# nyrahealth/CrisperWhisper

Hardware: AMD Instinct MI355X
Metric: aligned words/s (RTF alongside), CrisperWhisper large-v3 geometry, 30 s chunks, full mel->encoder->decoder->DTW->words path (higher is better)
Workload: dtype bf16

## Files before the change

crisperwhisper_amd/csrc/common.h:

```cpp
#pragma once
#include <hip/hip_runtime.h>
#include <stdint.h>
#include <stdio.h>
#include <math.h>

typedef unsigned short bf16_t;

typedef __attribute__((ext_vector_type(8))) short bf16x8_t;
typedef __attribute__((ext_vector_type(4))) float f32x4_t;

#define CW_WAVE 64

#ifdef CW_NO_NT
#define CW_STREAM_LD(p) (*(p))
#else
#define CW_STREAM_LD(p) __builtin_nontemporal_load(p)
#endif

static inline float cw_host_bf16_to_f32(unsigned short v) { union { uint32_t u; float f; } x; x.u = ((uint32_t)v) << 16; return x.f; }
static inline unsigned short cw_host_f32_to_bf16(float f) {
    union { uint32_t u; float f; } x; x.f = f;
    const uint32_t rounded = (x.u + 0x7fffu + ((x.u >> 16) & 1u)) >> 16;
    const uint32_t nan = (x.u >> 16) | 0x40u;
    return (unsigned short)(((x.u & 0x7fffffffu) > 0x7f800000u) ? nan : rounded);
// ... 268 lines not shown
        Pack4<T>::st((T*)p.out + (size_t)m * p.ldo + n, a0, a1, a2, a3);
    } else if (MODE == EPI_GELU) {
        Pack4<T>::st((T*)p.out + (size_t)m * p.ldo + n, Pack4<T>::gelu(a0), Pack4<T>::gelu(a1), Pack4<T>::gelu(a2), Pack4<T>::gelu(a3));
    } else if (MODE == EPI_RESID_F32) {
        const size_t o = (size_t)m * p.ldo + n;
        const float4 r = *(const float4*)(p.resid + o);
        *(float4*)(p.outf + o) = make_float4(r.x + a0, r.y + a1, r.z + a2, r.w + a3);
    } else if (MODE == EPI_GELU_POS_F32) {
        const float4 ps = *(const float4*)(p.pos + (size_t)(m % p.T) * p.ldo + n);
        *(float4*)(p.outf + (size_t)m * p.ldo + n) =
            make_float4(Pack4<T>::gelu(a0) + ps.x, Pack4<T>::gelu(a1) + ps.y, Pack4<T>::gelu(a2) + ps.z, Pack4<T>::gelu(a3) + ps.w);
    } else if (MODE == EPI_HEADS) {
        const int which = n / p.d_model, r = n - which * p.d_model;
        const int h = r >> 6, dd = r & 63;
        const int b = m / p.T, s = m - b * p.T;
        T* base = (T*)(which == 0 ? p.out : (which == 1 ? p.out1 : p.out2));
        Pack4<T>::st(base + (((size_t)b * p.H + h) * p.S_pad + s) * 64 + dd, a0, a1, a2, a3);
    } else if (MODE == EPI_STORE_F32) {
        *(float4*)(p.outf + (size_t)m * p.ldo + n) = make_float4(a0, a1, a2, a3);
    }
}

template <typename T, int MODE>
__device__ inline void epi_tile_interior(const EpiParams& p, const int (&rows)[4], const int (&cols)[4],
                                         const f32x4_t (&acc)[4][4]) {
    size_t roff[4]; int rpos[4];
    float4 bias[4]; size_t coff[4]; T* cbase[4];
#pragma unroll
    for (int i = 0; i < 4; ++i) {
        const int m = rows[i];
        rpos[i] = 0;
        if (MODE == EPI_HEADS) {
            const int b = m / p.T, s_ = m - b * p.T;
            roff[i] = ((size_t)b * p.H * p.S_pad + s_) * 64;
        } else {
            roff[i] = (size_t)m * p.ldo;
            if (MODE == EPI_GELU_POS_F32) rpos[i] = m % p.T;
        }
    }
#pragma unroll
    for (int j = 0; j < 4; ++j) {
        const int n = cols[j];
        bias[j] = p.bias ? *(const float4*)(p.bias + n) : make_float4(0.f, 0.f, 0.f, 0.f);
        cbase[j] = (T*)p.out;
        if (MODE == EPI_HEADS) {
            const int which = n / p.d_model, r = n - which * p.d_model;
            cbase[j] = (T*)(which == 0 ? p.out : (which == 1 ? p.out1 : p.out2));
            coff[j] = (size_t)(r >> 6) * p.S_pad * 64 + (r & 63);
        } else {
            coff[j] = (size_t)n;
        }
    }
#pragma unroll
    for (int i = 0; i < 4; ++i)
#pragma unroll
        for (int j = 0; j < 4; ++j) {
            const float a0 = acc[i][j][0] + bias[j].x, a1 = acc[i][j][1] + bias[j].y;
            const float a2 = acc[i][j][2] + bias[j].z, a3 = acc[i][j][3] + bias[j].w;
            const size_t o = roff[i] + coff[j];
            if (MODE == EPI_STORE || MODE == EPI_HEADS) {
                Pack4<T>::st(cbase[j] + o, a0, a1, a2, a3);
            } else if (MODE == EPI_GELU) {
                Pack4<T>::st(cbase[j] + o, Pack4<T>::gelu(a0), Pack4<T>::gelu(a1), Pack4<T>::gelu(a2), Pack4<T>::gelu(a3));
            } else if (MODE == EPI_RESID_F32) {
                const float4 r = *(const float4*)(p.resid + o);
                *(float4*)(p.outf + o) = make_float4(r.x + a0, r.y + a1, r.z + a2, r.w + a3);
            } else if (MODE == EPI_GELU_POS_F32) {
                const float4 ps = *(const float4*)(p.pos + (size_t)rpos[i] * p.ldo + cols[j]);
                *(float4*)(p.outf + o) = make_float4(Pack4<T>::gelu(a0) + ps.x, Pack4<T>::gelu(a1) + ps.y,
                                                     Pack4<T>::gelu(a2) + ps.z, Pack4<T>::gelu(a3) + ps.w);
            } else if (MODE == EPI_STORE_F32) {
                *(float4*)(p.outf + o) = make_float4(a0, a1, a2, a3);
            }
        }
}

#define CW_OK 0
#define CW_ERR_INVALID (-22)
#define CW_ERR_NOMEM (-12)
#define CW_ERR_HIP (-5)
#define CW_ERR_STATE (-1)
#define CW_TOP_LOGPROBS_MAX 8
```

crisperwhisper_amd/csrc/engine.hip:

```cpp
#include <chrono>
#include <hip/hip_runtime.h>
#include <stdarg.h>
#include <stdlib.h>
#include <string.h>
#include <set>
#include <string>
#include <vector>
#include <functional>
#include <algorithm>

#include "../../include/crisperwhisper.h"
#include "kernels.h"

static thread_local char g_err[512] = "";

#define KD(c, fn, ...) ((c)->f16 ? cw_f16::fn(__VA_ARGS__) : cw_bf16::fn(__VA_ARGS__))

#define CW_MAX_DEC_STAGES 24
enum DecStageKind { DST_OTHER = 0, DST_QKV_SELF, DST_QKV, DST_SELF_ATTN, DST_O_PROJ, DST_STACK, DST_STACK_CROSS, DST_CROSS_Q, DST_CROSS_ATTN,
                    DST_CROSS_O, DST_FC1, DST_FC2, DST_MLP_PAIR, DST_MLP_CHAIN, DST_N };
static const char* const kDecStageName[DST_N] = {
    "other (A/B path)", "LayerNorm + q/k/v projection + self-attention (qkv_self_kernel)", "LayerNorm + q/k/v projection + cache append",
    "self-attention", "self-attention out-projection", "fused out-projection + cross-query stage (gemv_stack_kernel)",
    "fused stage + cross-attention (dec_layer_a_kernel)", "LayerNorm + cross-attention query projection", "cross-attention",
// ... 50 lines not shown
    bool mid16 = true;
    bool dtw_block = false;
    bool stack_center = true;
    int skinny_mode = 0;
    float* d_planes = nullptr;
    size_t planes_cap = 0;
    float* d_sk_stats = nullptr;
    float* d_rstats = nullptr;
    bool fuse6_enabled = true;
    bool fuse_mlp = false;
    bool mlp_pair_fence = false;
    bool mlp_pair = false;
    unsigned int* d_bar = nullptr; int* d_err = nullptr;
    int handoff_fallbacks = 0;
    int handoff_resumes = 0;
    long long forwards_since_reset = 0;
    int fail_pos = -1;
    bool declayer = false;
    bool qkv_self = true;
    unsigned long long *d_gq = nullptr, *d_gps = nullptr, *d_gq2 = nullptr, *d_gkv = nullptr, *d_gflag = nullptr;
    bool mlp_chain = false;
    unsigned int* d_epoch = nullptr;
    int n_cu = 0;
    int stack_nt3 = 0, stack_nt5 = 0;
    bool ln_folded = false;
    bool fold_enabled = true;
    std::set<std::string> loaded;
    bool weights_ok = false;
    bool wpacked = false;
    bool wpack_enabled = true;
    void* embed_pk = nullptr;

    void *conv1_w = nullptr, *conv2_w = nullptr, *embed = nullptr;
    float *conv1_b = nullptr, *conv2_b = nullptr, *enc_pos = nullptr, *dec_pos = nullptr;
    float *enc_ln_g = nullptr, *enc_ln_b = nullptr, *dec_ln_g = nullptr, *dec_ln_b = nullptr;
    std::vector<LayerW> enc, dec;

    MelTables mel{};
    float *d_pcm = nullptr, *d_logspec = nullptr, *d_feats_hf = nullptr;
    unsigned int* d_gmax = nullptr;
    void* d_feats_tm = nullptr;
    std::vector<int> n_frames_items;

    void *c1 = nullptr, *h = nullptr, *qb = nullptr, *kb = nullptr, *vb = nullptr, *ao = nullptr, *mid = nullptr,
         *enc_out = nullptr;
    float* x = nullptr;
// ... 561 lines not shown
        "model.encoder.embed_positions.weight", "model.encoder.layer_norm.weight", "model.encoder.layer_norm.bias",
        "model.decoder.embed_tokens.weight", "model.decoder.embed_positions.weight", "model.decoder.layer_norm.weight",
        "model.decoder.layer_norm.bias"};
    auto attn = [&](const std::string& p) {
        for (const char* t : {".q_proj.weight", ".q_proj.bias", ".k_proj.weight", ".v_proj.weight", ".v_proj.bias",
                              ".out_proj.weight", ".out_proj.bias"}) want.push_back(p + t);
    };
    auto pair = [&](const std::string& p) { want.push_back(p + ".weight"); want.push_back(p + ".bias"); };
    for (int stack = 0; stack < 2; ++stack) {
        const int nl = stack ? c->d.dec_layers : c->d.enc_layers;
        for (int l = 0; l < nl; ++l) {
            const std::string p = std::string(stack ? "model.decoder.layers." : "model.encoder.layers.") + std::to_string(l);
            attn(p + ".self_attn"); pair(p + ".self_attn_layer_norm");
            if (stack) { attn(p + ".encoder_attn"); pair(p + ".encoder_attn_layer_norm"); }
            pair(p + ".fc1"); pair(p + ".fc2"); pair(p + ".final_layer_norm");
        }
    }
    std::string missing; int n_missing = 0;
    for (const auto& w : want)
        if (!c->loaded.count(w)) { if (n_missing < 4) missing += (n_missing ? ", " : "") + w; ++n_missing; }
    if (n_missing) return fail(c, CW_ERR_STATE, "%d of %zu weight tensors were never loaded (e.g. %s): incomplete checkpoint", n_missing, want.size(), missing.c_str());
    CWCHK(c, apply_folds(c));
    CWCHK(c, pack_decoder_weights(c));
    c->weights_ok = true;
    return CW_OK;
}

static int stage_fold(cw_ctx* c, int layer, int which, const float* data, int N, int K, void* w_dst, size_t w_off, float* b_dst,
                      size_t b_off, float scale) {
    cw_ctx::Fold f{nullptr, N, K, w_dst, w_off, b_dst, b_off, scale, layer, which};
    HIPCHK(c, hipMalloc((void**)&f.stage, (size_t)N * K * 4));
    HIPCHK(c, hipMemcpy(f.stage, data, (size_t)N * K * 4, hipMemcpyHostToDevice));
    c->folds.push_back(f);
    return CW_OK;
}

static int apply_folds(cw_ctx* c) {
    for (auto& f : c->folds) {
        LayerW& L = c->dec[f.layer];
        const float* g = f.which == 0 ? L.ln1_g : (f.which == 1 ? L.lnc_g : L.ln2_g);
        const float* b = f.which == 0 ? L.ln1_b : (f.which == 1 ? L.lnc_b : L.ln2_b);
        CWCHK(c, KD(c, cw_launch_fold_layernorm, f.stage, f.N, f.K, g, b, f.scale, (bf16_t*)f.w_dst + f.w_off, f.b_dst + f.b_off, c->st));
    }
    const int D = c->d.d_model, F = c->d.ffn_dim;
    bool all = !c->folds.empty() && c->fuse6_enabled && F % D == 0 && D <= 1280 && D % 64 == 0 && F % 64 == 0 && c->d.n_heads <= 20;
    if (all) {
// ... 287 lines not shown
        }
        if (c->enc8_mask & 2) CWCHK(c, KD(c, cw_launch_layernorm_fp8, c->x, L.ln2_g, L.ln2_b, c->h8, c->sa8, M, D, c->st));
        else CWCHK(c, KD(c, cw_launch_layernorm, bf, c->x, L.ln2_g, L.ln2_b, c->h, M, D, c->st));
        {
            AParams ap{c->h, D, 0, 0, 0, 0, nullptr, nullptr};
            EpiParams ep = epi0(); ep.out = c->mid; ep.bias = L.b1; ep.ldo = F;
            if (c->enc8_mask & 2) CWCHK(c, KD(c, cw_launch_gemm_fp8, EPI_GELU, c->h8, D, L.w18, M, F, D, c->sa8, L.s1, ep, c->st));
            else CWCHK(c, KD(c, cw_launch_gemm, bf, EPI_GELU, ap, L.w1, M, F, D, ep, c->st));
        }
        {
            AParams ap{c->mid, F, 0, 0, 0, 0, nullptr, nullptr};
            EpiParams ep = epi0(); ep.outf = c->x; ep.resid = c->x; ep.bias = L.b2; ep.ldo = D;
            if (c->enc8_mask & 4) {
                CWCHK(c, KD(c, cw_launch_quant_rows_fp8, c->mid, M, F, c->mid8, c->smid8, c->st));
                CWCHK(c, KD(c, cw_launch_gemm_fp8, EPI_RESID_F32, c->mid8, F, L.w28, M, D, F, c->smid8, L.s2, ep, c->st));
            } else CWCHK(c, KD(c, cw_launch_gemm, bf, EPI_RESID_F32, ap, L.w2, M, D, F, ep, c->st));
        }
    }
    CWCHK(c, KD(c, cw_launch_layernorm, bf, c->x, c->enc_ln_g, c->enc_ln_b, c->enc_out, M, D, c->st));
    if (c->enc8_mask & 8) CWCHK(c, KD(c, cw_launch_layernorm_fp8, c->x, c->enc_ln_g, c->enc_ln_b, c->h8, c->sa8, M, D, c->st));
    KCHK(c);
    tm.stop();
    StageTimer tk(c, CW_STAGE_CROSS_KV);
    for (int l = 0; l < c->d.dec_layers; ++l) {
        LayerW& L = c->dec[l];
        AParams ap{c->enc_out, D, 0, 0, 0, 0, nullptr, nullptr};
        EpiParams ep = epi0(); ep.out = L.ck; ep.out1 = L.cv; ep.bias = L.bkv_c;
        ep.T = S; ep.S_pad = S; ep.H = H; ep.d_model = D;
        if (c->enc8_mask & 8) CWCHK(c, KD(c, cw_launch_gemm_fp8, EPI_HEADS, c->h8, D, L.wkv_c8, M, 2 * D, D, c->sa8, L.skv_c, ep, c->st));
        else CWCHK(c, KD(c, cw_launch_gemm, bf, EPI_HEADS, ap, L.wkv_c, M, 2 * D, D, ep, c->st));
        if (c->kv8) CWCHK(c, KD(c, cw_launch_kv_quant_fp8, L.ck, L.cv, L.ck8, L.cv8, L.kvs, nb, H, S, c->st));
    }
    KCHK(c);
    tk.stop();
    c->nb_encoded = nb;
    return CW_OK;
}

int32_t cw_get_encoder_output(cw_ctx* c, float* out, int32_t nb) {
    if (nb < 1 || nb > c->nb_encoded) return fail(c, CW_ERR_STATE, "only %d windows encoded", c->nb_encoded);
    HIPCHK(c, hipStreamSynchronize(c->st));
    return download_T(c, c->enc_out, 0, out, (size_t)nb * CW_N_CTX * c->d.d_model);
}

static int gemv_ln(cw_ctx* c, int epi, const float* x, int Mb, int K, const void* W, int N, const float* g,
                   const float* b, const EpiParams& ep) {
    if (c->bf16 || !g) return KD(c, cw_launch_gemv, c->bf16, epi, x, Mb, K, W, N, g, b, ep, c->st, nullptr, (Mb <= 16 || c->wpacked) ? c->d_xfrag : nullptr, c->bf16 && c->wpacked);
// ... 1976 lines not shown
        for (auto& ge : c->step_graph) if (ge) { hipGraphExecDestroy(ge); ge = nullptr; }
        return CW_OK;
    }
    return fail(c, CW_ERR_INVALID, "unknown option %s", name);
}

int32_t cw_has_experiments(void) {
#ifdef CW_EXPERIMENTS
    return 1;
#else
    return 0;
#endif
}

static int g_test_cross_fp8 = 0;
static int g_test_attn_poison_qpad = 0;
int32_t cw_test_set_option(const char* name, int32_t value) {
    if (!strcmp(name, "cross_test_fp8")) { g_test_cross_fp8 = value; return CW_OK; }
    if (!strcmp(name, "attn_poison_qpad")) { g_test_attn_poison_qpad = value; return CW_OK; }
    if (!strcmp(name, "gemm256_min_tiles")) { cw_bf16::cw_gemm_set_256_min_tiles(value); cw_f16::cw_gemm_set_256_min_tiles(value); return CW_OK; }
    if (!strcmp(name, "beam_topk_1block")) { cw_bf16::cw_beam_topk_set_1block(value); cw_f16::cw_beam_topk_set_1block(value); return CW_OK; }
    if (!strcmp(name, "gemm_pp")) { cw_bf16::cw_gemm_set_pp(value); cw_f16::cw_gemm_set_pp(value); return CW_OK; }
    if (!strcmp(name, "gemm_8ph")) { cw_bf16::cw_gemm_set_8ph(value); cw_f16::cw_gemm_set_8ph(value); return CW_OK; }
    if (!strcmp(name, "gemm_gm")) {
#ifndef CW_EXPERIMENTS
        return CW_ERR_INVALID;
#endif
        cw_bf16::cw_gemm_set_gm(value); cw_f16::cw_gemm_set_gm(value); return CW_OK;
    }
    if (!strcmp(name, "gemv_loop")) { cw_bf16::cw_gemv_set_loop(value); cw_f16::cw_gemv_set_loop(value); return CW_OK; }
    if (!strcmp(name, "mt_variant")) { cw_bf16::cw_gemv_set_mt_variant(value); cw_f16::cw_gemv_set_mt_variant(value); return CW_OK; }
    if (!strcmp(name, "comb_rowgroups")) { cw_bf16::cw_gemv_set_comb_rowgroups(value); cw_f16::cw_gemv_set_comb_rowgroups(value); return CW_OK; }
    if (!strcmp(name, "gemm_w128")) { cw_bf16::cw_gemm_set_w128(value); cw_f16::cw_gemm_set_w128(value); return CW_OK; }
    if (!strcmp(name, "cross_valu")) { cw_bf16::cw_cross_set_valu(value); cw_f16::cw_cross_set_valu(value); return CW_OK; }
    if (!strcmp(name, "cross_per_row")) { cw_bf16::cw_cross_set_per_row(value); cw_f16::cw_cross_set_per_row(value); return CW_OK; }
    return CW_ERR_INVALID;
}

int32_t cw_test_gemm(cw_ctx* c, int32_t M, int32_t N, int32_t K, const float* A, const float* W, const float* bias,
                     int32_t gelu, float* out) {
    void *dA = nullptr, *dW = nullptr, *dO = nullptr; float* dB = nullptr;
    const size_t e = c->esz;
    HIPCHK(c, hipMalloc(&dA, (size_t)M * K * e)); HIPCHK(c, hipMalloc(&dW, (size_t)N * K * e));
    HIPCHK(c, hipMalloc(&dO, (size_t)M * N * e)); HIPCHK(c, hipMalloc((void**)&dB, (size_t)N * 4));
    CWCHK(c, upload_T(c, dA, 0, A, (size_t)M * K)); CWCHK(c, upload_T(c, dW, 0, W, (size_t)N * K));
    if (bias) HIPCHK(c, hipMemcpy(dB, bias, (size_t)N * 4, hipMemcpyHostToDevice));
// ... 1540 lines not shown
```

crisperwhisper_amd/csrc/gemm.hip:

```cpp
#include "common.h"
#include "kernels.h"
#include <stdlib.h>
#include <mutex>
#include "gemm_tiles.h"

namespace CW_NS {

#define BM 128
#define BN 128
#define LDS_STRIDE 72

typedef __attribute__((ext_vector_type(4))) unsigned int u32x4_t;

__device__ inline f32x4_t mfma16(bf16x8_t a, bf16x8_t b, f32x4_t c) { return cw_mfma_16x16x32(a, b, c); }

template <typename TA>
__device__ inline const TA* a_row_ptr(const AParams& ap, int m, int M, int k0) {
    if (m >= M) return nullptr;
    if (ap.amode == 0) return (const TA*)ap.A + (size_t)m * ap.lda + k0;
    int b = m / ap.T_out, t = m - b * ap.T_out;
    int tap = k0 / ap.C_in, c0 = k0 - tap * ap.C_in;
    int t_in = t * ap.stride + tap - 1;
    if (t_in < 0 || t_in >= ap.row_valid[b]) return nullptr;
    return (const TA*)ap.A + ((size_t)(ap.row_off[b] + t_in)) * ap.C_in + c0;
// ... 628 lines not shown
            epi_tile_interior<bf16_t, EPI>(ep, rows, cols, acc[h]);
        }
        return;
    }
#pragma unroll
    for (int h = 0; h < 2; ++h)
#pragma unroll
        for (int i = 0; i < 4; ++i) {
            const int m = m0 + h * 128 + wr * 64 + i * 16 + l15;
            if (m >= M) continue;
#pragma unroll
            for (int j = 0; j < 4; ++j) {
                const int n = cols[j];
                if (vec_ok) {
                    epi_store4<bf16_t, EPI>(ep, m, n, acc[h][i][j][0], acc[h][i][j][1], acc[h][i][j][2], acc[h][i][j][3]);
                } else {
#pragma unroll
                    for (int r = 0; r < 4; ++r) epi_store1<bf16_t, EPI>(ep, m, n + r, acc[h][i][j][r]);
                }
            }
        }
}

typedef __attribute__((ext_vector_type(8))) int i32x8_t;
__device__ inline i32x8_t frag_fp8(const unsigned char* row, int c_lo, int c_hi) {
    const u32x4_t lo = *(const u32x4_t*)(row + c_lo), hi = *(const u32x4_t*)(row + c_hi);
    return (i32x8_t){(int)lo[0], (int)lo[1], (int)lo[2], (int)lo[3], (int)hi[0], (int)hi[1], (int)hi[2], (int)hi[3]};
}

template <int EPI>
__global__ __launch_bounds__(512) void gemm_fp8_pp_kernel(const unsigned char* __restrict__ A, int lda,
                                                          const unsigned char* __restrict__ W, int M, int N, int K,
                                                          const float* __restrict__ sa, const float* __restrict__ sw,
                                                          EpiParams ep, int tiles_n) {
    extern __shared__ __attribute__((aligned(16))) unsigned char gsm4[];
    const int tid = threadIdx.x, lane = tid & 63;
    const int wave = __builtin_amdgcn_readfirstlane(tid >> 6);
    const int wm = wave >> 2, wn = wave & 3;
    const int l15 = lane & 15, g = lane >> 4;
    const int tile = xcd_remap(blockIdx.x, gridDim.x);
    int mt_, nt_;
    grouped_tile(tile, gridDim.x / tiles_n, tiles_n, mt_, nt_);
    const int m0 = mt_ * BM2, n0 = nt_ * BN2;

    const int lrow = lane >> 3;
    const int csrc = ((lane & 7) ^ lrow) * 16;
// ... 951 lines not shown
        for (int i = 0; i < 8; ++i) {
            float v = wave_sum(acc[i]);
            if (lane == 0 && mb + i < Mb) epi_store1<float, EPI>(ep, mb + i, n, v);
        }
    }
}

static const bf16_t* g_zero_page = nullptr;
static bool g_use_glds = true;
static bool g_use_256 = true;
static int g_256_min_tiles = 200;
static int g_use_pp = -1;
void cw_gemm_set_256_min_tiles(int n) { g_256_min_tiles = n; }
static int g_use_8ph = -1;
void cw_gemm_set_pp(int on) { g_use_pp = on; }
void cw_gemm_set_8ph(int on) { g_use_8ph = on; }
void cw_gemm_set_gm(int gm) {
#ifdef CW_EXPERIMENTS
    if (gm == 0) gm = 8;
    (void)hipMemcpyToSymbol(HIP_SYMBOL(c_gemm_gm), &gm, sizeof(int));
#else
    (void)gm;
#endif
}
static int g_gemv_loop = -1;
void cw_gemv_set_loop(int on) { g_gemv_loop = on; }
static int g_comb_rowgroups = -1;
void cw_gemv_set_comb_rowgroups(int on) { g_comb_rowgroups = on; }
static int g_use_w128 = -1;
void cw_gemm_set_w128(int on) { g_use_w128 = on; }

template <int EPI>
static void launch_gemm_epi(bool bf16, const AParams& ap, const void* W, int M, int N, int K, const EpiParams& ep,
                            hipStream_t st) {
    if (bf16) {
        int tm = (M + BM - 1) / BM, tn = (N + BN - 1) / BN;
        static std::once_flag once;
        std::call_once(once, [] {
            void* z = nullptr;
            if (hipMalloc(&z, 256) == hipSuccess) { hipMemset(z, 0, 256); g_zero_page = (const bf16_t*)z; }
            if (cw_sw::cw_switches().no_glds) g_use_glds = false;
            if (cw_sw::cw_switches().no_gemm256) g_use_256 = false;
        });
        const int tm2 = (M + BM2 - 1) / BM2, tn2 = (N + BN2 - 1) / BN2;
        if (g_use_pp < 0) g_use_pp = !cw_sw::cw_switches().no_gemm_pp;
        const bool use_pp = g_use_pp != 0;
        if (g_use_8ph < 0) g_use_8ph = !cw_sw::cw_switches().no_gemm_8ph;
#ifdef CW_EXPERIMENTS
        if (g_use_w128 < 0) g_use_w128 = cw_sw::cw_switches().gemm_w128;
#else
        g_use_w128 = 0;
#endif
        if (g_use_glds && g_zero_page && g_use_256 && g_use_w128 && tm2 * tn2 >= g_256_min_tiles && ap.amode == 0 && N % BN2 == 0) {
            cw_launch_gemm_w128(EPI, (const bf16_t*)ap.A, ap.lda, (const bf16_t*)W, M, N, K, ep, tm2, tn2, st);
        } else if (g_use_glds && g_zero_page && g_use_256 && use_pp && g_use_8ph && tm2 * tn2 >= g_256_min_tiles && ap.amode == 0 && N % BN2 == 0) {
            static std::once_flag attr_8;
            std::call_once(attr_8, [] {
                hipFuncSetAttribute((const void*)gemm_bf16_8ph_kernel<EPI>, hipFuncAttributeMaxDynamicSharedMemorySize, 131072);
            });
            hipLaunchKernelGGL((gemm_bf16_8ph_kernel<EPI>), dim3(tm2 * tn2), dim3(512), 131072, st, (const bf16_t*)ap.A, ap.lda,
                               (const bf16_t*)W, M, N, K, ep, tn2);
#ifdef CW_EXPERIMENTS
        } else if (g_use_glds && g_zero_page && g_use_256 && use_pp && tm2 * tn2 >= g_256_min_tiles && ap.amode == 0 && N % BN2 == 0) {
            static std::once_flag attr_pp;
            std::call_once(attr_pp, [] {
                hipFuncSetAttribute((const void*)gemm_bf16_pp_kernel<EPI>, hipFuncAttributeMaxDynamicSharedMemorySize, 131072);
            });
            hipLaunchKernelGGL((gemm_bf16_pp_kernel<EPI>), dim3(tm2 * tn2), dim3(512), 131072, st, (const bf16_t*)ap.A, ap.lda,
                               (const bf16_t*)W, M, N, K, ep, tn2, g_zero_page);
#endif
        } else if (g_use_glds && g_zero_page && g_use_256 && tm2 * tn2 >= g_256_min_tiles) {
            static std::once_flag attr_once;
            std::call_once(attr_once, [] {
                hipFuncSetAttribute((const void*)gemm_bf16_256_kernel<EPI>, hipFuncAttributeMaxDynamicSharedMemorySize, 131072);
            });
            hipLaunchKernelGGL((gemm_bf16_256_kernel<EPI>), dim3(tm2 * tn2), dim3(512), 131072, st, ap, (const bf16_t*)W, M,
                               N, K, ep, tn2, g_zero_page);
        } else if (g_use_glds && g_zero_page)
            hipLaunchKernelGGL((gemm_bf16_glds_kernel<EPI>), dim3(tm * tn), dim3(256), 65536, st, ap, (const bf16_t*)W, M,
                               N, K, ep, tn, g_zero_page);
        else
        hipLaunchKernelGGL((gemm_bf16_kernel<EPI>), dim3(tm * tn), dim3(256), 0, st, ap, (const bf16_t*)W, M, N, K, ep,
                           tn);
    } else {
        int tm = (M + 63) / 64, tn = (N + 63) / 64;
        hipLaunchKernelGGL((gemm_f32_kernel<EPI>), dim3(tm * tn), dim3(256), 0, st, ap, (const float*)W, M, N, K, ep,
                           tn);
    }
}

int cw_launch_gemm(bool bf16, int epi, const AParams& ap, const void* W, int M, int N, int K, const EpiParams& ep,
                   hipStream_t st) {
    if (K % 64 != 0 || M <= 0 || N <= 0) return CW_ERR_INVALID;
    switch (epi) {
        case EPI_STORE: launch_gemm_epi<EPI_STORE>(bf16, ap, W, M, N, K, ep, st); break;
        case EPI_GELU: launch_gemm_epi<EPI_GELU>(bf16, ap, W, M, N, K, ep, st); break;
        case EPI_RESID_F32: launch_gemm_epi<EPI_RESID_F32>(bf16, ap, W, M, N, K, ep, st); break;
        case EPI_GELU_POS_F32: launch_gemm_epi<EPI_GELU_POS_F32>(bf16, ap, W, M, N, K, ep, st); break;
        case EPI_HEADS: launch_gemm_epi<EPI_HEADS>(bf16, ap, W, M, N, K, ep, st); break;
        case EPI_STORE_F32: launch_gemm_epi<EPI_STORE_F32>(bf16, ap, W, M, N, K, ep, st); break;
        default: return CW_ERR_INVALID;
    }
    return CW_OK;
}

int cw_launch_quant_rows_fp8(const void* x, int rows, int K, void* out8, float* scale, hipStream_t st) {
    if (K % 8 != 0 || rows <= 0) return CW_ERR_INVALID;
    hipLaunchKernelGGL(quant_rows_fp8_kernel, dim3((rows + 3) / 4), dim3(256), 0, st, (const bf16_t*)x, rows, K, (unsigned char*)out8, scale);
    return CW_OK;
}

template <int EPI>
static void launch_gemm_fp8_epi(const void* A8, int lda, const void* W8, int M, int N, int K, const float* sa, const float* sw,
                                const EpiParams& ep, hipStream_t st) {
    static std::once_flag attr_once;
    std::call_once(attr_once, [] {
        hipFuncSetAttribute((const void*)gemm_fp8_pp_kernel<EPI>, hipFuncAttributeMaxDynamicSharedMemorySize, 131072);
    });
    const int tm2 = (M + BM2 - 1) / BM2, tn2 = N / BN2;
    hipLaunchKernelGGL((gemm_fp8_pp_kernel<EPI>), dim3(tm2 * tn2), dim3(512), 131072, st, (const unsigned char*)A8, lda,
                       (const unsigned char*)W8, M, N, K, sa, sw, ep, tn2);
}

int cw_launch_gemm_fp8(int epi, const void* A8, int lda, const void* W8, int M, int N, int K, const float* sa, const float* sw,
                       const EpiParams& ep, hipStream_t st) {
// ... 353 lines not shown
```

crisperwhisper_amd/csrc/kernels.h:

```cpp
#pragma once
#include "switches.h"
#include "common.h"

struct AParams {
    const void* A;
    int lda;
    int amode;
    int T_out, C_in, stride;
    const int* row_off;
    const int* row_valid;
};

struct CombineParams;


struct SampleParams {
    const float* logits;
    int V, B, ldv;
    const unsigned char* mask;
    int eos, pad, timestamp_begin, max_initial_timestamp_index;
    const int* cfg;
    int* pos;
    int ids_stride;
    int* ids;
// ... 264 lines not shown
    void* out;
    float* x;
    void* sk; void* sv;
    int D, H, cap, n_pos;
};
struct PrefillAlign {
    float* out;
    float* ml;
    const int* slot;
    int n_align, rows;
};

struct ScorePart {
    float mx, sum;
    float tl;
    float bv; int bi;
};

#define CW_DTYPE_KERNEL_DECLS \
    int cw_launch_gemm(bool bf16, int epi, const AParams& ap, const void* W, int M, int N, int K, const EpiParams& ep, hipStream_t st); \
    void cw_gemm_set_256_min_tiles(int n); \
    void cw_gemm_set_pp(int on); \
    void cw_gemm_set_8ph(int on); \
    void cw_gemm_set_gm(int gm); \
    void cw_gemm_set_w128(int on); \
    void cw_gemv_set_comb_rowgroups(int on); \
    void cw_gemv_set_mt_variant(int v); \
    void cw_gemv_set_loop(int on); \
    int cw_launch_gemm_w128(int epi, const bf16_t* A, int lda, const bf16_t* W, int M, int N, int K, const EpiParams& ep, int tm2, int tn2, hipStream_t st); \
    void cw_cross_set_valu(int on); \
    void cw_cross_set_per_row(int on); \
    int cw_launch_layernorm_fp8(const float* x, const float* g, const float* b, void* out8, float* scale, int rows, int d, hipStream_t st); \
    int cw_launch_quant_rows_fp8(const void* x, int rows, int K, void* out8, float* scale, hipStream_t st); \
    int cw_launch_gemm_fp8(int epi, const void* A8, int lda, const void* W8, int M, int N, int K, const float* sa, const float* sw, const EpiParams& ep, hipStream_t st); \
    int cw_launch_fold_layernorm(const float* Wf, int N, int K, const float* g, const float* beta, float scale, void* w_out, float* bias, hipStream_t st); \
    int cw_launch_gemv(bool bf16, int epi, const float* x, int Mb, int K, const void* W, int N, const float* ln_g, const float* ln_b, const EpiParams& ep, hipStream_t st, const CombineParams* comb = nullptr, void* scratch = nullptr, bool wpacked = false); \
    int cw_gemv_own_nt(int N); \
    int cw_launch_gemv_own(const void* xf, int Mb, int K, const void* W, int N, const EpiParams& ep, const float* cvec, void* xf_out, float* stats_out, hipStream_t st, bool wpacked); \
    int cw_launch_gemv_lna(const void* xf, int Mb, int K, const void* W, int N, const EpiParams& ep, const float* stats_in, int n_stats, const float* wsum, hipStream_t st, bool wpacked); \
    size_t cw_wfrag_elems(int N, int K); \
    int cw_launch_wfrag_pack(const void* src, int N, int K, void* dst, hipStream_t st); \
    int cw_launch_fold_product(const float* A, const float* s, float scale, const float* B, int N, int J, int K, void* C16, hipStream_t st); \
    int cw_launch_fold_rowvec(const float* A, const float* s, float scale, const float* v, const void* W16, int N, int J, float* c_out, float* w_out, hipStream_t st); \
    int cw_launch_gemv_stack(const StackParams& p, int nt, hipStream_t st); \
    int cw_launch_dec_layer(const DecLayerParams& p, int n_cu, hipStream_t st); \
    bool cw_mlp_chain_ok(int Mb, int D, int F); \
// ... 62 lines not shown
```

crisperwhisper_amd/csrc/switches.cpp:

```cpp
#include "switches.h"
#include <cstdlib>

namespace cw_sw {

static bool flag(const char* name) { return getenv(name) != nullptr; }
static int num(const char* name, int dflt) { const char* v = getenv(name); return v ? atoi(v) : dflt; }

Switches read_switches() {
    Switches s{};
    s.no_graph = flag("CW_NO_GRAPH");
    s.no_ln_fold = flag("CW_NO_LN_FOLD");
    s.no_fuse6 = flag("CW_NO_FUSE6");
    s.rows_ln = flag("CW_ROWS_LN");
    s.no_rows_hilo = flag("CW_NO_ROWS_HILO");
    s.no_stack_center = flag("CW_NO_STACK_CENTER");
    s.no_mid16 = flag("CW_NO_MID16");
    s.dtw_block = flag("CW_DTW_BLOCK");
    s.fuse_mlp = flag("CW_FUSE_MLP");
    s.no_wpack = flag("CW_NO_WPACK");
    s.mlp_pair = flag("CW_MLP_PAIR");
    s.mlp_pair_fence = flag("CW_MLP_PAIR_FENCE");
    s.declayer = flag("CW_DECLAYER");
    s.no_qkv_self = flag("CW_NO_QKV_SELF");
    s.mlp_chain = flag("CW_MLP_CHAIN");
// ... 5 lines not shown
    s.skinny = num("CW_SKINNY", 0);
    s.prefetch = num("CW_PREFETCH", 0);
    s.prefetch_wide = num("CW_PREFETCH_WIDE", 0);
    s.prefetch_what = num("CW_PREFETCH_WHAT", 3);
    s.stack_nt3 = num("CW_STACK_NT3", 0);
    s.stack_nt5 = num("CW_STACK_NT5", 0);
    s.attn_v1 = flag("CW_ATTN_V1");
    s.anc_attn_v1 = flag("CW_ANC_ATTN_V1");
    s.cross_per_row = flag("CW_CROSS_PER_ROW");
    s.cross_valu = flag("CW_CROSS_VALU");
    s.cross_no_tr = flag("CW_CROSS_NO_TR");
    s.cross8_valu = flag("CW_CROSS8_VALU");
    s.cross_mfma1 = flag("CW_CROSS_MFMA1");
    s.cross_lds_pad = num("CW_CROSS_LDS_PAD", 0);
    s.cross8_nsb = num("CW_CROSS8_NSB", 0);
    s.dl_depth = num("CW_DL_DEPTH", 16);
    s.dl_kvwait = num("CW_DL_KVWAIT", 0);
    s.mlp_chain_delay = num("CW_MLP_CHAIN_DELAY", 0);
    s.qkv_self_dbg = num("CW_QKV_SELF_DBG", 0);
    s.no_glds = flag("CW_NO_GLDS");
    s.no_gemm256 = flag("CW_NO_GEMM256");
    s.no_gemm_pp = flag("CW_NO_GEMM_PP");
    s.no_gemm_8ph = flag("CW_NO_GEMM_8PH");
    s.gemm_w128 = flag("CW_GEMM_W128");
    s.no_gemv_loop = flag("CW_NO_GEMV_LOOP");
    s.comb_nt2 = flag("CW_COMB_NT2");
    s.comb_no_rowgroups = flag("CW_COMB_NO_ROWGROUPS");
    s.comb_g4 = flag("CW_COMB_G4");
    s.mt_no_prea = flag("CW_MT_NO_PREA");
    s.gemv_loop_cap = num("CW_GEMV_LOOP_CAP", 512);
    s.fc2_ksplit = num("CW_FC2_KSPLIT", 0);
    s.mt_variant = num("CW_MT_VARIANT", -1);
    s.own_nt = num("CW_OWN_NT", 1);
    if (s.mt_variant < -1 || s.mt_variant > 2) s.mt_variant = -1;
    s.beam_topk_1block = flag("CW_BEAM_TOPK_1BLOCK");
    s.mel_valu = flag("CW_MEL_VALU");
    s.mel_dbg = num("CW_MEL_DBG", 0);
    s.test_gemm_reps = num("CW_TEST_GEMM_REPS", 0);
    s.test_attn_reps = num("CW_TEST_ATTN_REPS", 0);
    if (s.gemv_loop_cap < 1) s.gemv_loop_cap = 1;
    if (s.fc2_ksplit < 0) s.fc2_ksplit = 0;
    if (s.cross_lds_pad < 0) s.cross_lds_pad = 0;
    if (s.cross_lds_pad > 150 * 1024) s.cross_lds_pad = 150 * 1024;
    if (s.stack_nt3 < 0 || s.stack_nt3 > 3) s.stack_nt3 = 0;
    if (s.stack_nt5 < 0 || s.stack_nt5 > 3) s.stack_nt5 = 0;
    if (s.prefetch < 0) s.prefetch = 0;
// ... 13 lines not shown
```

crisperwhisper_amd/csrc/switches.h:

```cpp
#pragma once

namespace cw_sw {

struct Switches {
    bool no_graph, no_ln_fold, no_fuse6, rows_ln, no_rows_hilo, no_stack_center, no_mid16, dtw_block, fuse_mlp, no_wpack, mlp_pair, mlp_pair_fence, declayer, no_qkv_self, mlp_chain, no_fuse_rows, no_fuse_rows8, no_fuse_beam, no_own_cols, no_short_hist;
    int skinny, prefetch, prefetch_wide, prefetch_what, stack_nt3, stack_nt5;
    bool attn_v1, anc_attn_v1, cross_per_row, cross_valu, cross_no_tr, cross8_valu, cross_mfma1;
    int cross_lds_pad, cross8_nsb, dl_depth, dl_kvwait, mlp_chain_delay, qkv_self_dbg;
    bool no_glds, no_gemm256, no_gemm_pp, no_gemm_8ph, gemm_w128, no_gemv_loop, comb_nt2, comb_no_rowgroups, mt_no_prea, comb_g4;
    int gemv_loop_cap, fc2_ksplit, mt_variant, own_nt;
    bool beam_topk_1block, mel_valu;
    int mel_dbg;
    int test_gemm_reps, test_attn_reps;
};

const Switches& cw_switches();
Switches read_switches();

}
```

Before: 754.8.

## Add persistent tile-walking GEMM and grouped cross-KV projection across decoder layers

Adds a persistent variant of the 8-phase bf16 GEMM kernel that walks several output tiles per block and prefetches the next tile's operands while the current tile's epilogue runs. The per-layer cross-attention K/V projections are replaced by one grouped launch over all decoder layers, with per-layer weights, biases and outputs read from a device-side table. This cuts launch count and tail-wave idle time on the cross-KV stage. It adds code complexity, a kernel-local bias hoist, and a risk that the grid capped at the CU count leaves bandwidth unused or balances poorly.

After: 754.6. Within noise of the previous version (-0.0%).

```diff
diff --git a/crisperwhisper_amd/csrc/common.h b/crisperwhisper_amd/csrc/common.h
--- a/crisperwhisper_amd/csrc/common.h
+++ b/crisperwhisper_amd/csrc/common.h
@@ -314,10 +314,10 @@
 }
 
 template <typename T, int MODE>
-__device__ inline void epi_tile_interior(const EpiParams& p, const int (&rows)[4], const int (&cols)[4],
-                                         const f32x4_t (&acc)[4][4]) {
+__device__ inline void epi_tile_interior_b(const EpiParams& p, const int (&rows)[4], const int (&cols)[4],
+                                           const float4 (&bias)[4], const f32x4_t (&acc)[4][4]) {
     size_t roff[4]; int rpos[4];
-    float4 bias[4]; size_t coff[4]; T* cbase[4];
+    size_t coff[4]; T* cbase[4];
 #pragma unroll
     for (int i = 0; i < 4; ++i) {
         const int m = rows[i];
@@ -333,7 +333,6 @@
 #pragma unroll
     for (int j = 0; j < 4; ++j) {
         const int n = cols[j];
-        bias[j] = p.bias ? *(const float4*)(p.bias + n) : make_float4(0.f, 0.f, 0.f, 0.f);
         cbase[j] = (T*)p.out;
         if (MODE == EPI_HEADS) {
             const int which = n / p.d_model, r = n - which * p.d_model;
@@ -367,6 +366,67 @@
         }
 }
 
+template <typename T, int MODE>
+__device__ inline void epi_tile_interior(const EpiParams& p, const int (&rows)[4], const int (&cols)[4],
+                                         const f32x4_t (&acc)[4][4]) {
+    size_t roff[4]; int rpos[4];
+    float4 bias[4]; size_t coff[4]; T* cbase[4];
+#pragma unroll
+    for (int i = 0; i < 4; ++i) {
+        const int m = rows[i];
+        rpos[i] = 0;
+        if (MODE == EPI_HEADS) {
+            const int b = m / p.T, s_ = m - b * p.T;
+            roff[i] = ((size_t)b * p.H * p.S_pad + s_) * 64;
+        } else {
+            roff[i] = (size_t)m * p.ldo;
+            if (MODE == EPI_GELU_POS_F32) rpos[i] = m % p.T;
+        }
+    }
+#pragma unroll
+    for (int j = 0; j < 4; ++j) {
+        const int n = cols[j];
+        bias[j] = p.bias ? *(const float4*)(p.bias + n) : make_float4(0.f, 0.f, 0.f, 0.f);
+        cbase[j] = (T*)p.out;
+        if (MODE == EPI_HEADS) {
+            const int which = n / p.d_model, r = n - which * p.d_model;
+            cbase[j] = (T*)(which == 0 ? p.out : (which == 1 ? p.out1 : p.out2));
+            coff[j] = (size_t)(r >> 6) * p.S_pad * 64 + (r & 63);
+        } else {
+            coff[j] = (size_t)n;
+        }
+    }
+#pragma unroll
+    for (int i = 0; i < 4; ++i)
+#pragma unroll
+        for (int j = 0; j < 4; ++j) {
+            const float a0 = acc[i][j][0] + bias[j].x, a1 = acc[i][j][1] + bias[j].y;
+            const float a2 = acc[i][j][2] + bias[j].z, a3 = acc[i][j][3] + bias[j].w;
+            const size_t o = roff[i] + coff[j];
+            if (MODE == EPI_STORE || MODE == EPI_HEADS) {
+                Pack4<T>::st(cbase[j] + o, a0, a1, a2, a3);
+            } else if (MODE == EPI_GELU) {
+                Pack4<T>::st(cbase[j] + o, Pack4<T>::gelu(a0), Pack4<T>::gelu(a1), Pack4<T>::gelu(a2), Pack4<T>::gelu(a3));
+            } else if (MODE == EPI_RESID_F32) {
+                const float4 r = *(const float4*)(p.resid + o);
+                *(float4*)(p.outf + o) = make_float4(r.x + a0, r.y + a1, r.z + a2, r.w + a3);
+            } else if (MODE == EPI_GELU_POS_F32) {
+                const float4 ps = *(const float4*)(p.pos + (size_t)rpos[i] * p.ldo + cols[j]);
+                *(float4*)(p.outf + o) = make_float4(Pack4<T>::gelu(a0) + ps.x, Pack4<T>::gelu(a1) + ps.y,
+                                                     Pack4<T>::gelu(a2) + ps.z, Pack4<T>::gelu(a3) + ps.w);
+            } else if (MODE == EPI_STORE_F32) {
+                *(float4*)(p.outf + o) = make_float4(a0, a1, a2, a3);
+            }
+        }
+}
+
+struct GemmGroup {
+    const void* W;
+    const float* bias;
+    void* out;
+    void* out1;
+};
+
 #define CW_OK 0
 #define CW_ERR_INVALID (-22)
 #define CW_ERR_NOMEM (-12)
diff --git a/crisperwhisper_amd/csrc/engine.hip b/crisperwhisper_amd/csrc/engine.hip
--- a/crisperwhisper_amd/csrc/engine.hip
+++ b/crisperwhisper_amd/csrc/engine.hip
@@ -96,6 +96,7 @@
     bool mlp_chain = false;
     unsigned int* d_epoch = nullptr;
     int n_cu = 0;
+    GemmGroup* d_ckv_grp = nullptr;
     int stack_nt3 = 0, stack_nt5 = 0;
     bool ln_folded = false;
     bool fold_enabled = true;
@@ -703,6 +704,12 @@
     if (n_missing) return fail(c, CW_ERR_STATE, "%d of %zu weight tensors were never loaded (e.g. %s): incomplete checkpoint", n_missing, want.size(), missing.c_str());
     CWCHK(c, apply_folds(c));
     CWCHK(c, pack_decoder_weights(c));
+    {
+        std::vector<GemmGroup> grp;
+        for (auto& L : c->dec) grp.push_back(GemmGroup{L.wkv_c, L.bkv_c, L.ck, L.cv});
+        if (!c->d_ckv_grp) CWCHK(c, dmalloc(c, &c->d_ckv_grp, grp.size() * sizeof(GemmGroup)));
+        HIPCHK(c, hipMemcpy(c->d_ckv_grp, grp.data(), grp.size() * sizeof(GemmGroup), hipMemcpyHostToDevice));
+    }
     c->weights_ok = true;
     return CW_OK;
 }
@@ -1036,7 +1043,14 @@
     KCHK(c);
     tm.stop();
     StageTimer tk(c, CW_STAGE_CROSS_KV);
-    for (int l = 0; l < c->d.dec_layers; ++l) {
+    int grouped = 1;
+    if (bf && !(c->enc8_mask & 8) && !c->kv8 && c->d.dec_layers > 0) {
+        EpiParams ep = epi0();
+        ep.T = S; ep.S_pad = S; ep.H = H; ep.d_model = D;
+        grouped = KD(c, cw_launch_gemm_grouped_heads, c->enc_out, D, c->d_ckv_grp, c->d.dec_layers, M, 2 * D, D, ep, c->st);
+        if (grouped < 0) CWCHK(c, grouped);
+    }
+    for (int l = 0; l < (grouped ? c->d.dec_layers : 0); ++l) {
         LayerW& L = c->dec[l];
         AParams ap{c->enc_out, D, 0, 0, 0, 0, nullptr, nullptr};
         EpiParams ep = epi0(); ep.out = L.ck; ep.out1 = L.cv; ep.bias = L.bkv_c;
@@ -3059,6 +3073,7 @@
     if (!strcmp(name, "beam_topk_1block")) { cw_bf16::cw_beam_topk_set_1block(value); cw_f16::cw_beam_topk_set_1block(value); return CW_OK; }
     if (!strcmp(name, "gemm_pp")) { cw_bf16::cw_gemm_set_pp(value); cw_f16::cw_gemm_set_pp(value); return CW_OK; }
     if (!strcmp(name, "gemm_8ph")) { cw_bf16::cw_gemm_set_8ph(value); cw_f16::cw_gemm_set_8ph(value); return CW_OK; }
+    if (!strcmp(name, "gemm_persist")) { cw_bf16::cw_gemm_set_persist(value); cw_f16::cw_gemm_set_persist(value); return CW_OK; }
     if (!strcmp(name, "gemm_gm")) {
 #ifndef CW_EXPERIMENTS
         return CW_ERR_INVALID;
diff --git a/crisperwhisper_amd/csrc/gemm.hip b/crisperwhisper_amd/csrc/gemm.hip
--- a/crisperwhisper_amd/csrc/gemm.hip
+++ b/crisperwhisper_amd/csrc/gemm.hip
@@ -674,6 +674,242 @@
         }
 }
 
+template <int EPI, bool GROUPED>
+__global__ __launch_bounds__(512) void gemm_bf16_8ph_walk_kernel(const bf16_t* __restrict__ A, int lda, const bf16_t* W, int M, int N, int K,
+                                                            EpiParams ep, int tiles_n, int ntiles,
+                                                            const GemmGroup* __restrict__ grp, int group_tiles) {
+    extern __shared__ __attribute__((aligned(16))) unsigned char gsm4[];
+    const int tid = threadIdx.x, lane = tid & 63;
+    const int wave = __builtin_amdgcn_readfirstlane(tid >> 6);
+    const int wr = wave >> 2, wn = wave & 3;
+    const int l15 = lane & 15, g = lane >> 4;
+
+    const int lrow = lane >> 3;
+    const int csrc = ((lane & 7) ^ lrow) * 8;
+    const __amdgpu_buffer_rsrc_t ra = __builtin_amdgcn_make_buffer_rsrc((void*)A, (short)0, 0x7fffffff, 0x00020000);
+    int m0 = 0, n0 = 0, grp_i = 0;
+    const bf16_t* Wt = W;
+    int va[2][2], vw = 0;
+    auto set_tile = [&](int lt) {
+#ifdef CW_EXPERIMENTS
+        const int gm_ = c_gemm_gm;
+        int tile = gm_ < 0 ? lt : xcd_remap(lt, ntiles);
+#else
+        int tile = xcd_remap(lt, ntiles);
+#endif
+        int per = ntiles;
+        if constexpr (GROUPED) {
+            per = group_tiles;
+            grp_i = tile / per;
+            tile -= grp_i * per;
+            Wt = (const bf16_t*)grp[grp_i].W;
+        }
+        int mt_, nt_;
+#ifdef CW_EXPERIMENTS
+        grouped_tile(tile, per / tiles_n, tiles_n, mt_, nt_, gm_ < 0 ? -gm_ : gm_);
+#else
+        grouped_tile(tile, per / tiles_n, tiles_n, mt_, nt_);
+#endif
+        m0 = mt_ * BM2; n0 = nt_ * BN2;
+#pragma unroll
+        for (int h = 0; h < 2; ++h)
+#pragma unroll
+            for (int q = 0; q < 2; ++q) va[h][q] = (min(m0 + h * 128 + wave * 16 + q * 8 + lrow, M - 1) * lda + csrc) * 2;
+        vw = ((n0 + wave * 16 + lrow) * K + csrc) * 2;
+    };
+    auto issue_a = [&](int k0, int buf, int h) {
+#ifdef CW_8PH_NO_DMA
+        return;
+#endif
+        unsigned char* base = gsm4 + buf * 65536 + (h * 128 + wave * 16) * 128;
+#pragma unroll
+        for (int q = 0; q < 2; ++q)
+            __builtin_amdgcn_raw_ptr_buffer_load_lds(ra, (__attribute__((address_space(3))) void*)(base + q * 1024), 16, va[h][q], k0 * 2, 0, 0);
+    };
+    auto issue_w = [&](int k0, int buf, int h) {
+#ifdef CW_8PH_NO_DMA
+        return;
+#endif
+        const __amdgpu_buffer_rsrc_t rw = __builtin_amdgcn_make_buffer_rsrc((void*)Wt, (short)0, 0x7fffffff, 0x00020000);
+        unsigned char* base = gsm4 + buf * 65536 + 32768 + (h * 128 + wave * 16) * 128;
+#pragma unroll
+        for (int q = 0; q < 2; ++q)
+            __builtin_amdgcn_raw_ptr_buffer_load_lds(rw, (__attribute__((address_space(3))) void*)(base + q * 1024), 16, vw,
+                                                     (k0 + (h * 128 + q * 8) * K) * 2, 0, 0);
+    };
+    const int sw = l15 & 7;
+    const int aoff = (wr * 64 + l15) * 128, woff = 32768 + (wn * 32 + l15) * 128;
+    bf16x8_t fa[2][4], fw[2][2][2];
+    auto read_a = [&](int buf, int h) {
+#ifdef CW_8PH_NO_READS
+        if (buf >= 0) return;
+#endif
+        const unsigned char* sb = gsm4 + buf * 65536 + aoff + h * 16384;
+#pragma unroll
+        for (int kk = 0; kk < 2; ++kk) {
+            const int c = ((kk * 4 + g) ^ sw) << 4;
+#pragma unroll
+            for (int i = 0; i < 4; ++i) fa[kk][i] = *(const bf16x8_t*)(sb + i * 2048 + c);
+        }
+    };
+    auto read_w = [&](int buf, int h) {
+#ifdef CW_8PH_NO_READS
+        if (buf >= 0) return;
+#endif
+        const unsigned char* sb = gsm4 + buf * 65536 + woff + h * 16384;
+#pragma unroll
+        for (int kk = 0; kk < 2; ++kk) {
+            const int c = ((kk * 4 + g) ^ sw) << 4;
+#pragma unroll
+            for (int j = 0; j < 2; ++j) fw[h][kk][j] = *(const bf16x8_t*)(sb + j * 2048 + c);
+        }
+    };
+    f32x4_t acc[2][4][4];
+#define CW_8PH_COMPUTE(hm, hn)                                                                              \
+    do {                                                                                                    \
+        __builtin_amdgcn_s_barrier();                                                                       \
+        asm volatile("s_waitcnt lgkmcnt(0)" ::: "memory");                                                  \
+        __builtin_amdgcn_sched_barrier(0);                                                                  \
+        __builtin_amdgcn_s_setprio(1);                                                                      \
+        _Pragma("unroll") for (int kk = 0; kk < 2; ++kk)                                                    \
+            _Pragma("unroll") for (int i = 0; i < 4; ++i)                                                   \
+                _Pragma("unroll") for (int j = 0; j < 2; ++j)                                               \
+                    acc[hm][i][(hn) * 2 + j] = mfma16(fw[hn][kk][j], fa[kk][i], acc[hm][i][(hn) * 2 + j]); \
+        __builtin_amdgcn_s_setprio(0);                                                                      \
+        __builtin_amdgcn_sched_barrier(0);                                                                  \
+        __builtin_amdgcn_s_barrier();                                                                       \
+    } while (0)
+#ifndef CW_8PH_VMCNT
+#define CW_8PH_VMCNT 6
+#endif
+#define CW_8PH_STR2(x) #x
+#define CW_8PH_STR(x) CW_8PH_STR2(x)
+#define CW_8PH_WAIT(steady)                                                                                 \
+    do {                                                                                                    \
+        if (steady) asm volatile("s_waitcnt vmcnt(" CW_8PH_STR(CW_8PH_VMCNT) ")" ::: "memory");             \
+        else asm volatile("s_waitcnt vmcnt(0)" ::: "memory");                                               \
+        __builtin_amdgcn_sched_barrier(0);                                                                  \
+    } while (0)
+
+    const int nk = K / BK;
+    auto prologue = [&]() {
+        issue_a(0, 0, 0); issue_w(0, 0, 0); issue_w(0, 0, 1); issue_a(0, 0, 1);
+        if (nk > 1) issue_a(BK, 1, 0);
+    };
+    const bool vec_ok = (EPI == EPI_HEADS || (ep.ldo & 3) == 0);
+    float4 nbias[4];
+    auto load_bias = [&]() {
+        const float* bp = ep.bias;
+        if constexpr (GROUPED) bp = grp[grp_i].bias;
+#pragma unroll
+        for (int j = 0; j < 4; ++j) {
+            const int col = n0 + (j >> 1) * 128 + wn * 32 + (j & 1) * 16 + g * 4;
+            nbias[j] = bp ? *(const float4*)(bp + col) : make_float4(0.f, 0.f, 0.f, 0.f);
+        }
+    };
+    int lt = blockIdx.x;
+    bool seam_counted = false;
+    set_tile(lt);
+    load_bias();
+    __builtin_amdgcn_sched_barrier(0);
+    prologue();
+    for (;;) {
+#pragma unroll
+        for (int h = 0; h < 2; ++h)
+#pragma unroll
+            for (int i = 0; i < 4; ++i)
+#pragma unroll
+                for (int j = 0; j < 4; ++j) acc[h][i][j] = (f32x4_t){0.f, 0.f, 0.f, 0.f};
+        if (seam_counted) asm volatile("s_waitcnt vmcnt(16)" ::: "memory");
+        else asm volatile("s_waitcnt vmcnt(0)" ::: "memory");
+        __builtin_amdgcn_sched_barrier(0);
+#pragma unroll
+        for (int j = 0; j < 4; ++j) asm volatile("" : "+v"(nbias[j].x), "+v"(nbias[j].y), "+v"(nbias[j].z), "+v"(nbias[j].w));
+        __builtin_amdgcn_s_barrier();
+        if (wr == 1) __builtin_amdgcn_s_barrier();
+        for (int t = 0; t < nk; ++t) {
+            const int b = t & 1, nb = b ^ 1;
+            const bool nxt = t + 1 < nk, nxt2 = t + 2 < nk;
+            const bool steady = t + 2 < nk;
+            const int k1 = (t + 1) * BK, k2 = (t + 2) * BK;
+            read_w(b, 0);
+            __builtin_amdgcn_sched_barrier(0);
+            read_a(b, 0);
+            __builtin_amdgcn_sched_barrier(0);
+            if (nxt) issue_w(k1, nb, 0);
+            CW_8PH_WAIT(steady);
+            CW_8PH_COMPUTE(0, 0);
+            read_w(b, 1);
+            __builtin_amdgcn_sched_barrier(0);
+            if (nxt) issue_w(k1, nb, 1);
+            CW_8PH_WAIT(steady);
+            CW_8PH_COMPUTE(0, 1);
+            read_a(b, 1);
+            __builtin_amdgcn_sched_barrier(0);
+            if (nxt) issue_a(k1, nb, 1);
+            CW_8PH_WAIT(steady);
+            CW_8PH_COMPUTE(1, 1);
+            if (nxt2) issue_a(k2, b, 0);
+            CW_8PH_WAIT(steady);
+            CW_8PH_COMPUTE(1, 0);
+        }
+        if (wr == 0) __builtin_amdgcn_s_barrier();
+
+        const int em0 = m0, en0 = n0;
+        EpiParams epl = ep;
+        if constexpr (GROUPED) { epl.bias = grp[grp_i].bias; epl.out = grp[grp_i].out; epl.out1 = grp[grp_i].out1; }
+        const int nlt = lt + (int)gridDim.x;
+        const bool more = nlt < ntiles;
+        const bool interior = em0 + BM2 <= M && vec_ok;
+        int cols[4];
+#pragma unroll
+        for (int j = 0; j < 4; ++j) cols[j] = en0 + (j >> 1) * 128 + wn * 32 + (j & 1) * 16 + g * 4;
+        float4 bias[4];
+#pragma unroll
+        for (int j = 0; j < 4; ++j) bias[j] = nbias[j];
+        __builtin_amdgcn_sched_barrier(0);
+        if (more) {
+            set_tile(nlt);
+            load_bias();
+            __builtin_amdgcn_sched_barrier(0);
+            prologue();
+        }
+        __builtin_amdgcn_sched_barrier(0);
+        if (interior) {
+#pragma unroll
+            for (int h = 0; h < 2; ++h) {
+                int rows[4];
+#pragma unroll
+                for (int i = 0; i < 4; ++i) rows[i] = em0 + h * 128 + wr * 64 + i * 16 + l15;
+                epi_tile_interior_b<bf16_t, EPI>(epl, rows, cols, bias, acc[h]);
+            }
+        } else {
+#pragma unroll
+            for (int h = 0; h < 2; ++h)
+#pragma unroll
+                for (int i = 0; i < 4; ++i) {
+                    const int m = em0 + h * 128 + wr * 64 + i * 16 + l15;
+                    if (m >= M) continue;
+#pragma unroll
+                    for (int j = 0; j < 4; ++j) {
+                        const int n = cols[j];
+                        if (vec_ok) {
+                            epi_store4<bf16_t, EPI>(epl, m, n, acc[h][i][j][0], acc[h][i][j][1], acc[h][i][j][2], acc[h][i][j][3]);
+                        } else {
+#pragma unroll
+                            for (int r = 0; r < 4; ++r) epi_store1<bf16_t, EPI>(epl, m, n + r, acc[h][i][j][r]);
+                        }
+                    }
+                }
+        }
+        if (!more) break;
+        lt = nlt;
+        seam_counted = interior;
+    }
+#undef CW_8PH_COMPUTE
+#undef CW_8PH_WAIT
+}
+
 typedef __attribute__((ext_vector_type(8))) int i32x8_t;
 __device__ inline i32x8_t frag_fp8(const unsigned char* row, int c_lo, int c_hi) {
     const u32x4_t lo = *(const u32x4_t*)(row + c_lo), hi = *(const u32x4_t*)(row + c_hi);
@@ -1671,6 +1907,17 @@
 #else
     (void)gm;
 #endif
+}
+static int g_use_persist = -1;
+void cw_gemm_set_persist(int on) { g_use_persist = on; }
+static int gemm_walk_grid(int tiles) {
+    static int n_cu = [] {
+        int dev = 0, n = 0;
+        if (hipGetDevice(&dev) != hipSuccess || hipDeviceGetAttribute(&n, hipDeviceAttributeMultiprocessorCount, dev) != hipSuccess) n = 0;
+        return n;
+    }();
+    if (g_use_persist < 0) g_use_persist = !cw_sw::cw_switches().no_gemm_persist;
+    return (n_cu > 0 && tiles > n_cu) ? n_cu : tiles;
 }
 static int g_gemv_loop = -1;
 void cw_gemv_set_loop(int on) { g_gemv_loop = on; }
@@ -1706,7 +1953,13 @@
             static std::once_flag attr_8;
             std::call_once(attr_8, [] {
                 hipFuncSetAttribute((const void*)gemm_bf16_8ph_kernel<EPI>, hipFuncAttributeMaxDynamicSharedMemorySize, 131072);
+                hipFuncSetAttribute((const void*)gemm_bf16_8ph_walk_kernel<EPI, false>, hipFuncAttributeMaxDynamicSharedMemorySize, 131072);
             });
+            const int grid = gemm_walk_grid(tm2 * tn2);
+            if (g_use_persist >= 2 && grid < tm2 * tn2)
+                hipLaunchKernelGGL((gemm_bf16_8ph_walk_kernel<EPI, false>), dim3(grid), dim3(512), 131072, st, (const bf16_t*)ap.A, ap.lda,
+                                   (const bf16_t*)W, M, N, K, ep, tn2, tm2 * tn2, (const GemmGroup*)nullptr, 0);
+            else
             hipLaunchKernelGGL((gemm_bf16_8ph_kernel<EPI>), dim3(tm2 * tn2), dim3(512), 131072, st, (const bf16_t*)ap.A, ap.lda,
                                (const bf16_t*)W, M, N, K, ep, tn2);
 #ifdef CW_EXPERIMENTS
@@ -1750,6 +2003,30 @@
         case EPI_STORE_F32: launch_gemm_epi<EPI_STORE_F32>(bf16, ap, W, M, N, K, ep, st); break;
         default: return CW_ERR_INVALID;
     }
+    return CW_OK;
+}
+
+int cw_launch_gemm_grouped_heads(const void* A, int lda, const GemmGroup* grp, int groups, int M, int N, int K, const EpiParams& ep,
+                                 hipStream_t st) {
+    if (K % 64 != 0 || M <= 0 || N <= 0 || groups < 1 || !grp) return CW_ERR_INVALID;
+    const int tm2 = (M + BM2 - 1) / BM2, tn2 = (N + BN2 - 1) / BN2;
+    if (g_use_pp < 0) g_use_pp = !cw_sw::cw_switches().no_gemm_pp;
+    if (g_use_8ph < 0) g_use_8ph = !cw_sw::cw_switches().no_gemm_8ph;
+    if (g_use_persist < 0) g_use_persist = !cw_sw::cw_switches().no_gemm_persist;
+    const auto& sw = cw_sw::cw_switches();
+#ifdef CW_EXPERIMENTS
+    if (g_use_w128 < 0) g_use_w128 = sw.gemm_w128;
+    if (g_use_w128) return 1;
+#endif
+    if (sw.no_glds || sw.no_gemm256 || !g_use_pp || !g_use_8ph || !g_use_persist || tm2 * tn2 < g_256_min_tiles || N % BN2 != 0 ||
+        (long long)groups * tm2 * tn2 > 0x3fffffff) return 1;
+    static std::once_flag attr_g;
+    std::call_once(attr_g, [] {
+        hipFuncSetAttribute((const void*)gemm_bf16_8ph_walk_kernel<EPI_HEADS, true>, hipFuncAttributeMaxDynamicSharedMemorySize, 131072);
+    });
+    const int per = tm2 * tn2, total = groups * per;
+    hipLaunchKernelGGL((gemm_bf16_8ph_walk_kernel<EPI_HEADS, true>), dim3(gemm_walk_grid(total)), dim3(512), 131072, st, (const bf16_t*)A, lda,
+                       (const bf16_t*)nullptr, M, N, K, ep, tn2, total, grp, per);
     return CW_OK;
 }
 
diff --git a/crisperwhisper_amd/csrc/kernels.h b/crisperwhisper_amd/csrc/kernels.h
--- a/crisperwhisper_amd/csrc/kernels.h
+++ b/crisperwhisper_amd/csrc/kernels.h
@@ -310,6 +310,8 @@
     void cw_gemm_set_256_min_tiles(int n); \
     void cw_gemm_set_pp(int on); \
     void cw_gemm_set_8ph(int on); \
+    void cw_gemm_set_persist(int on); \
+    int cw_launch_gemm_grouped_heads(const void* A, int lda, const GemmGroup* grp, int groups, int M, int N, int K, const EpiParams& ep, hipStream_t st); \
     void cw_gemm_set_gm(int gm); \
     void cw_gemm_set_w128(int on); \
     void cw_gemv_set_comb_rowgroups(int on); \
diff --git a/crisperwhisper_amd/csrc/switches.cpp b/crisperwhisper_amd/csrc/switches.cpp
--- a/crisperwhisper_amd/csrc/switches.cpp
+++ b/crisperwhisper_amd/csrc/switches.cpp
@@ -51,6 +51,7 @@
     s.no_gemm256 = flag("CW_NO_GEMM256");
     s.no_gemm_pp = flag("CW_NO_GEMM_PP");
     s.no_gemm_8ph = flag("CW_NO_GEMM_8PH");
+    s.no_gemm_persist = flag("CW_NO_GEMM_PERSIST");
     s.gemm_w128 = flag("CW_GEMM_W128");
     s.no_gemv_loop = flag("CW_NO_GEMV_LOOP");
     s.comb_nt2 = flag("CW_COMB_NT2");
diff --git a/crisperwhisper_amd/csrc/switches.h b/crisperwhisper_amd/csrc/switches.h
--- a/crisperwhisper_amd/csrc/switches.h
+++ b/crisperwhisper_amd/csrc/switches.h
@@ -7,7 +7,7 @@
     int skinny, prefetch, prefetch_wide, prefetch_what, stack_nt3, stack_nt5;
     bool attn_v1, anc_attn_v1, cross_per_row, cross_valu, cross_no_tr, cross8_valu, cross_mfma1;
     int cross_lds_pad, cross8_nsb, dl_depth, dl_kvwait, mlp_chain_delay, qkv_self_dbg;
-    bool no_glds, no_gemm256, no_gemm_pp, no_gemm_8ph, gemm_w128, no_gemv_loop, comb_nt2, comb_no_rowgroups, mt_no_prea, comb_g4;
+    bool no_glds, no_gemm256, no_gemm_pp, no_gemm_8ph, no_gemm_persist, gemm_w128, no_gemv_loop, comb_nt2, comb_no_rowgroups, mt_no_prea, comb_g4;
     int gemv_loop_cap, fc2_ksplit, mt_variant, own_nt;
     bool beam_topk_1block, mel_valu;
     int mel_dbg;
```
